# OthmanB/TAMCMC-C

Measured on AMD Instinct MI355X. Metric: MCMC samples/sec (whole node), 1e5 nu-bins x 100 params x 20 tempered chains, higher is better.
Workload: dtype f64

## Files before the change

### tamcmc-c_amd/csrc/dev_sampler.hip

```cpp
#include <hip/hip_runtime.h>

#include <atomic>
#include <chrono>
#include <hip/hip_ext.h>

#include <cmath>
#include <cstdio>
#include <cstdlib>
#include <cstring>
#include <algorithm>
#include <type_traits>
#include <utility>
#include <vector>

#include "ctx.h"
#include "rgb_prestep.h"
#include "dev_sampler.h"
#include "kernels.h"
#include "loglike_tile.h"
#include "dev_unpack.h"
#include "fd_batch.h"
#include "mode_tables.h"
#include "rng.h"
#include "step_schedule.h"

namespace tamcmc {

namespace {

#include "dev_iterate_impl.h"
#include "dev_step_impl.h"
#include "dev_mala_impl.h"

}


struct DevSampler::Impl {
    tamcmc_hip_ctx *ctx = nullptr;
    DevSamplerArgs a{};
    std::vector<void *> allocs;
    hipEvent_t ev[64][2];
    int n_ev = 0;
    bool poly_ready = false;
    double *adapt_scratch = nullptr;
    size_t smp_cap = 0, stat_cap = 0;
    size_t lds_base = 0, lds_adapt = 0;
    int parity = 0;
    FusedArgs f{};
    unsigned char *d_argcopy = nullptr;
    std::vector<unsigned char> h_argcopy;
    bool use_drift = false;
    double delta = 0, fd_step_rel = 1e-7;
    FdBatch fd;
    DevBuf<unsigned char> fd_block;
    DevBuf<double> fd_part, fd_S, fd_model, fd_bg;
    DevBuf<double> fused_bg, fused_part;
    MalaArgs mala{};
    bool grad_valid = false;
    int prior_class = 0, model_id = 0;
    std::vector<double> h_priors, h_extra;
    std::vector<int32_t> h_idx, h_sw;
    long armed_it = -1;
    int armed_q = 0;
    long it_fused = 0, it_lockstep = 0;
    long n_stretch = 0;
    int mala_chol_lds = -1;

    hipEvent_t gev[8][2];
    int n_gev = 0;
    bool rgb = false;
    int rgb_bmax = 0;
    bool fused_ok = false;
    int fused_mode = -1, fused_K = 0;
    int tile_rot = 0;
    std::vector<int32_t> h_plength;
    int G = 1;
    hipStream_t gst[4] = {nullptr, nullptr, nullptr, nullptr};
    hipEvent_t ev_kb[4], ev_ki[4], ev_fork, ev_join[4];
    bool ev_made = false;
    double *d_pack = nullptr, *h_pack = nullptr;

    double *device_view(const double *host, size_t bytes) {
        if (!host || !bytes) return nullptr;
        double *d = nullptr;
        void *dp = nullptr, *dq = nullptr;
        const char *last = (const char *)host + bytes - 1;
        if (hipHostGetDevicePointer(&dp, const_cast<double *>(host), 0) == hipSuccess && dp &&
            hipHostGetDevicePointer(&dq, const_cast<char *>(last), 0) == hipSuccess && dq == (char *)dp + bytes - 1)
            d = (double *)dp;
        else (void)hipGetLastError();
        return d;
    }

    static hipError_t wait_stream(hipStream_t st, bool poll) {
        const auto t0 = std::chrono::steady_clock::now();
        for (int spin = 0; poll; spin++) {
            const hipError_t e = hipStreamQuery(st);
            if (e != hipErrorNotReady) return e;
            if ((spin & 63) == 63 && std::chrono::steady_clock::now() - t0 > std::chrono::microseconds(1000)) break;
        }
        (void)hipGetLastError();
        return hipStreamSynchronize(st);
    }

    template <typename T>
    hipError_t dalloc(T **p, size_t n) {
        void *q = nullptr;
        hipError_t e = hipMalloc(&q, (n ? n : 1) * sizeof(T));
        if (e == hipSuccess) { allocs.push_back(q); *p = (T *)q; }
        return e;
    }

    struct KernelTiming;
    struct RunCall;
};

DevSampler::DevSampler() : impl(new Impl()) {}
DevSampler::~DevSampler() {
    if (!impl) return;
    if (impl->ctx) {
        (void)hipSetDevice(impl->ctx->device);
        (void)hipStreamSynchronize(impl->ctx->stream);
        for (int g = 1; g < 4; g++) if (impl->gst[g]) (void)hipStreamSynchronize(impl->gst[g]);
    }
#ifdef TAMCMC_PROBE
    if (impl->a.counters && getenv("TAMCMC_PROBE_STEP")) {
        long h[40];
        (void)hipMemcpy(h, impl->a.counters + 8 + impl->a.C, sizeof h, hipMemcpyDeviceToHost);
        if (h[35] > 0) fprintf(stderr, "build_multiplet, row 20 (us): decode + widths/heights %.2f | window %.2f | m loop %.2f\n", 0.01 * h[32] / h[35], 0.01 * h[33] / h[35], 0.01 * h[34] / h[35]);
        for (int r = 0; r < 4; r++)
            if (h[8 * r + 3] > 0)
                fprintf(stderr, "candidate role %d of slot 2 (us): decide %.2f | vectors + L z %.2f | role %.2f  [inside: %.2f | %.2f]  (%ld launches)\n", r,
                        0.01 * h[8 * r] / h[8 * r + 3], 0.01 * h[8 * r + 1] / h[8 * r + 3], 0.01 * h[8 * r + 2] / h[8 * r + 3],
                        0.01 * h[8 * r + 4] / h[8 * r + 3], 0.01 * h[8 * r + 5] / h[8 * r + 3], h[8 * r + 3]);
    }
    if (impl->a.counters && getenv("TAMCMC_PROBE_ADAPT")) {
        long h[8];
        (void)hipMemcpy(h, impl->a.counters, sizeof h, hipMemcpyDeviceToHost);
        if (h[7] > 0)
            fprintf(stderr, "Cholesky panels of chain 0 (us per panel): columns below %.2f | next panel's columns %.2f | next diagonal block beside the rest of the trailing update %.2f  (%ld panels)\n",
                    0.01 * h[4] / h[7], 0.01 * h[5] / h[7], 0.01 * h[6] / h[7], h[7]);
    }
#endif
    for (void *p : impl->allocs) (void)hipFree(p);
    impl->fd_block.release(); impl->fd_part.release(); impl->fd_S.release(); impl->fd_model.release(); impl->fd_bg.release(); impl->fused_bg.release(); impl->fused_part.release();
    if (impl->h_pack) (void)hipHostFree(impl->h_pack);
    for (int i = 0; i < impl->n_ev; i++) { (void)hipEventDestroy(impl->ev[i][0]); (void)hipEventDestroy(impl->ev[i][1]); }
    for (int i = 0; i < impl->n_gev; i++) { (void)hipEventDestroy(impl->gev[i][0]); (void)hipEventDestroy(impl->gev[i][1]); }
    if (impl->ev_made) {
        (void)hipEventDestroy(impl->ev_fork);
        for (int g = 0; g < 4; g++) { (void)hipEventDestroy(impl->ev_kb[g]); (void)hipEventDestroy(impl->ev_ki[g]); (void)hipEventDestroy(impl->ev_join[g]); }
        for (int g = 1; g < 4; g++) if (impl->gst[g]) (void)hipStreamDestroy(impl->gst[g]);
    }
    delete impl;
}

#define DCHK(call)                                                                   \
    do {                                                                             \
        hipError_t e_ = (call);                                                      \
        if (e_ != hipSuccess) {                                                      \
            c->err = std::string(#call) + ": " + hipGetErrorString(e_);              \
            return TAMCMC_ERR_HIP;                                                   \
        }                                                                            \
    } while (0)

template <typename T>
static hipError_t up(T *dst, const T *src, size_t n, hipStream_t st) {
    return hipMemcpyAsync(dst, src, n * sizeof(T), hipMemcpyHostToDevice, st);
}

int DevSampler::init(tamcmc_hip_ctx *c, const DevSamplerInit &in) {
    Impl &I = *impl;
    I.ctx = c;
    if (c->Nx <= 0) return TAMCMC_ERR_NO_SPECTRUM;
    if (in.C < 1 || in.C > TAMCMC_MAX_CHAINS) return TAMCMC_ERR_BAD_ARG;
    DCHK(hipSetDevice(c->device));
    DevSamplerArgs &a = I.a;
    a.desc.model_id = in.model_id; a.desc.prior_class = in.prior_class; a.C = in.C; a.desc.Np = in.Np; a.Nv = in.Nv;
    I.rgb = is_rgb_model(in.model_id);
#ifdef TAMCMC_PROBE
    if (const char *ep = getenv("TAMCMC_PROBE_ADAPT")) a.probe = atoi(ep);
#endif
    a.desc.per = I.rgb ? 0 : mt::count_multiplets(in.model_id, in.plength);
    I.h_plength.assign(in.plength, in.plength + 11);
    I.use_drift = in.use_drift != 0; I.delta = in.delta; I.fd_step_rel = in.fd_step_rel > 0 ? in.fd_step_rel : 1e-7;
    I.prior_class = in.prior_class; I.model_id = in.model_id;
    I.h_priors.assign(in.priors, in.priors + 4 * (size_t)in.Np); I.h_extra.assign(in.extra_priors, in.extra_priors + 10);
    I.h_idx.assign(in.index_to_relax, in.index_to_relax + in.Nv); I.h_sw.assign(in.priors_switch, in.priors_switch + in.Np);
    if (a.desc.per < 0) return TAMCMC_ERR_BAD_MODEL;
    a.desc.stride = in.plength[8] > 0 ? in.plength[8] : 1;
    if ((a.desc.stride - 1) / 3 > TAMCMC_MAX_HARVEY) return TAMCMC_ERR_BAD_ARG;
    {
        int G = in.chain_groups > 0 ? in.chain_groups : (in.C >= 8 ? 2 : 1);
        if (in.chain_groups <= 0 && I.rgb && in.C >= 16) G = 4;
        if (G > 4) G = 4;
        if (G > in.C) G = in.C;
        I.G = G;
    }
// ... 34 lines not shown
    DCHK(I.dalloc(&a.noise, CD * (size_t)a.desc.stride));
    DCHK(hipMemsetAsync(a.counters, 0, (8 + C + 64) * sizeof(long), st));
    DCHK(hipMemsetAsync(a.moved, 0, C * sizeof(int), st));
    DCHK(hipMemsetAsync(a.Pmove, 0, C * sizeof(double), st));
    a.samples = nullptr; a.stats = nullptr;
    I.lds_base = (Np + 2 * Nv + 1) * sizeof(double) + unpack_lds_bytes() + 32;
    I.lds_adapt = (Nv * Nv + Nv) * sizeof(double);
    a.chol_in_lds = (I.lds_base + I.lds_adapt <= 150 * 1024) ? 1 : 0;
    if (!a.chol_in_lds) { DCHK(I.dalloc(&I.adapt_scratch, C * (Nv * Nv + Nv))); I.lds_adapt = 0; }
    if (I.lds_base + I.lds_adapt > 64 * 1024) {
        DCHK(hipFuncSetAttribute((const void *)k_iterate<true>, hipFuncAttributeMaxDynamicSharedMemorySize, (int)(I.lds_base + I.lds_adapt)));
        DCHK(hipFuncSetAttribute((const void *)k_iterate<false>, hipFuncAttributeMaxDynamicSharedMemorySize, (int)(I.lds_base + I.lds_adapt)));
    }
    mt::PolyTab *d_tab;
    DCHK(I.dalloc(&d_tab, 1));
    hipLaunchKernelGGL(k_fill_poly, dim3(1), dim3(64), 0, st, d_tab);
    DCHK(hipGetLastError());
    a.desc.poly = d_tab;
    for (int i = 0; i < 64; i++) { DCHK(hipEventCreate(&I.ev[i][0])); DCHK(hipEventCreate(&I.ev[i][1])); I.n_ev = i + 1; }
    for (int i = 0; i < 8; i++) { DCHK(hipEventCreate(&I.gev[i][0])); DCHK(hipEventCreate(&I.gev[i][1])); I.n_gev = i + 1; }
    {
        const int G = I.G;
        I.gst[0] = st;
        for (int g = 1; g < G; g++) DCHK(hipStreamCreateWithFlags(&I.gst[g], hipStreamNonBlocking));
        DCHK(hipEventCreateWithFlags(&I.ev_fork, hipEventDisableTiming));
        for (int g = 0; g < 4; g++) {
            DCHK(hipEventCreateWithFlags(&I.ev_kb[g], hipEventDisableTiming));
            DCHK(hipEventCreateWithFlags(&I.ev_ki[g], hipEventDisableTiming));
            DCHK(hipEventCreateWithFlags(&I.ev_join[g], hipEventDisableTiming));
        }
        I.ev_made = true;
    }
    {
        FusedArgs &f = I.f;
        f.NS = 2 * in.C + 8;
        {
            const int h = (int)(((long)in.C * 1) / 2);
            f.xsplit = (I.G == 2 && h >= 3 && in.C - h >= 3) ? h : in.C;
        }
        const size_t NS = (size_t)f.NS;
        DCHK(I.dalloc(&f.cand_vars, 3 * NS * Nv)); DCHK(I.dalloc(&f.cand_params, 3 * NS * Np)); DCHK(I.dalloc(&f.cand_logPr, 6 * NS));
        DCHK(I.dalloc(&f.cand_stP, 6 * NS)); DCHK(I.dalloc(&f.cand_stR, 3 * NS)); DCHK(I.dalloc(&f.cand_rej, 3 * NS));
        DCHK(I.dalloc(&f.mults, 3 * NS * (size_t)a.desc.per + 1)); DCHK(I.dalloc(&f.pairs, 6 * NS)); DCHK(I.dalloc(&f.nh, 3 * NS)); DCHK(I.dalloc(&f.nn, 3 * NS));
        DCHK(I.dalloc(&f.noise, 3 * NS * (size_t)a.desc.stride));
        DCHK(I.dalloc(&f.slot, 2 * C)); DCHK(I.dalloc(&f.prop_logPr, 2 * C)); DCHK(I.dalloc(&f.prop_st, 2 * C)); DCHK(I.dalloc(&f.quick, 2 * C * QN)); DCHK(I.dalloc(&f.lz, 2 * C * Nv));
        DCHK(I.dalloc(&f.qcount, 2));
        DCHK(hipMemsetAsync(f.qcount, 0, 2 * sizeof(unsigned long long), st));
        f.qmargin = 1e-11;
        DCHK(hipMemsetAsync(f.nn, 0, 3 * NS * sizeof(int), st));
        DCHK(hipMemsetAsync(f.cand_stP, 0, 6 * NS * sizeof(int), st));
        DCHK(hipMemsetAsync(f.cand_rej, 0, 3 * NS * sizeof(int), st));
        DCHK(hipMemsetAsync(f.cand_stR, 0, 3 * NS * sizeof(int), st));
        f.part = nullptr;
        f.bg = nullptr;
        const size_t role_lds = (Np + 2 * Nv + 1) * sizeof(double) + unpack_lds_bytes() + 32;
        I.fused_ok = !I.rgb && role_lds <= sizeof(tile::TileLds<tile::M_FAST_DIRECT, 64>);
    }
    DCHK(hipStreamSynchronize(st));
    return TAMCMC_OK;
}

int DevSampler::download_gradient(double *grad, double *grad_prior) {
    Impl &I = *impl;
    tamcmc_hip_ctx *c = I.ctx;
    if (!I.use_drift || !I.a.grad_cur || !I.grad_valid) return TAMCMC_ERR_BAD_ARG;
    DCHK(hipSetDevice(c->device));
    const size_t n = (size_t)I.a.C * I.a.Nv;
    DCHK(hipStreamSynchronize(c->stream));
    if (grad) DCHK(hipMemcpy(grad, I.a.grad_cur + (size_t)I.parity * n, n * sizeof(double), hipMemcpyDeviceToHost));
    if (grad_prior) DCHK(hipMemcpy(grad_prior, I.a.gradP_cur + (size_t)I.parity * n, n * sizeof(double), hipMemcpyDeviceToHost));
    return TAMCMC_OK;
}

int DevSampler::download_last_proposal(double *vars_prop, double *grad_prop) {
    Impl &I = *impl;
    tamcmc_hip_ctx *c = I.ctx;
    if (!I.use_drift) return TAMCMC_ERR_BAD_ARG;
    DCHK(hipSetDevice(c->device));
    const size_t n = (size_t)I.a.C * I.a.Nv;
    DCHK(hipStreamSynchronize(c->stream));
    if (vars_prop) DCHK(hipMemcpy(vars_prop, I.a.vars_prop, n * sizeof(double), hipMemcpyDeviceToHost));
    if (grad_prop) DCHK(hipMemcpy(grad_prop, I.mala.grad_prop, n * sizeof(double), hipMemcpyDeviceToHost));
    return TAMCMC_OK;
}

void DevSampler::info(long out[11]) const {
    const Impl &I = *impl;
    unsigned long long qc[2] = {0, 0};
    if (I.f.qcount && hipSetDevice(I.ctx->device) == hipSuccess) (void)hipMemcpy(qc, I.f.qcount, sizeof qc, hipMemcpyDeviceToHost);
    out[8] = I.n_stretch; out[9] = (long)qc[0]; out[10] = (long)qc[1];
    out[0] = I.a.Nv; out[1] = I.a.desc.Np;
    out[2] = I.use_drift ? I.mala_chol_lds : I.a.chol_in_lds;
    out[3] = (I.fused_ok && !I.use_drift) ? 1 : 0;
    out[4] = I.G; out[5] = I.it_fused; out[6] = I.it_lockstep; out[7] = I.a.C;
}

int DevSampler::upload_state(const double *vars, const double *params, const double *logL, const double *logPr,
                             const double *logPost, const double *init_logL) {
    Impl &I = *impl;
    I.armed_it = -1;
    I.grad_valid = false;
    tamcmc_hip_ctx *c = I.ctx;
    DevSamplerArgs &a = I.a;
    const size_t C = (size_t)a.C, Np = (size_t)a.desc.Np, Nv = (size_t)a.Nv;
    hipStream_t st = c->stream;
    DCHK(hipSetDevice(c->device));
// ... 204 lines not shown
    return e;
}

struct DevSampler::Impl::RunCall {
    Impl &I;
    tamcmc_hip_ctx *c;
    DevSamplerArgs &a;
    const long it0, n_iter;
    const char *learn;
    double *samples, *stats;
    hipStream_t st;
    CallTimeline &tl;
    KernelTiming T;
    DevSamplerArgs args;
    LoglikeArgs la[4], lf[3];
    int goff[5];
    double *zc_smp = nullptr, *zc_st = nullptr;
    bool use_fused = false;
    bool split_ok = false;
    int P;
    StepCtl sc{};
    int q = 0;
    bool s1_must_wait = false;
    bool s1_ahead = false;
    bool s1_open = false;

    RunCall(Impl &I_, CallTimeline &tl_, long it0_, long n_iter_, const char *learn_, double *samples_, double *stats_)
        : I(I_), c(I_.ctx), a(I_.a), it0(it0_), n_iter(n_iter_), learn(learn_), samples(samples_), stats(stats_), st(I_.ctx->stream),
          tl(tl_), T{I_, I_.ctx}, P(I_.parity) {}

    int prepare() {
        const size_t C = (size_t)a.C, Nv = (size_t)a.Nv;
        const int tb = tile_bins(c->wgs, c->K);
        a.ntiles = (a.desc.Nx + tb - 1) / tb;
        DCHK(c->d_part.reserve(C * (size_t)a.ntiles * 2));
        a.partials = c->d_part.p;
        a.tile_bins = tb;
        a.bg = nullptr;
        use_fused = I.fused_ok && c->step_scheme != 1 && c->wgs == 64 && (c->K == 4 || c->K == 8 || c->K == 16);
        I.f.qmargin = c->quick_decide == 1 ? (double)INFINITY : 1e-11;
        const size_t NS = (size_t)I.f.NS;
        I.f.bg = nullptr;
        if (c->precision == TAMCMC_PRECISION_FAST) {
            DCHK(c->d_bg.reserve(C * (size_t)a.ntiles * 8));
            a.bg = c->d_bg.p;
            if (use_fused) {
                DCHK(I.fused_bg.reserve(3 * NS * (size_t)a.ntiles * 8));
                I.f.bg = I.fused_bg.p;
            }
        }
        if (use_fused) {
            DCHK(I.fused_part.reserve(2 * C * (size_t)a.ntiles * 2));
            I.f.part = I.fused_part.p;
        }
        split_ok = I.f.xsplit < a.C && c->step_scheme != 2 && (c->step_scheme == 3 || (long)a.C * a.ntiles >= 2500);
        auto grown = [](size_t need, size_t have, size_t unit) { const size_t floor_ = 256 * unit; return std::max(std::max(need, floor_), have * 2); };
        zc_smp = I.device_view(samples, (size_t)n_iter * C * Nv * 8);
        zc_st = I.device_view(stats, (size_t)n_iter * C * 3 * 8);
        if (samples && !zc_smp && I.smp_cap < (size_t)n_iter * C * Nv) {
            const size_t cap = grown((size_t)n_iter * C * Nv, I.smp_cap, C * Nv);
            DCHK(I.dalloc(&a.samples, cap));
            I.smp_cap = cap;
        }
        if (stats && !zc_st && I.stat_cap < (size_t)n_iter * C * 3) {
            const size_t cap = grown((size_t)n_iter * C * 3, I.stat_cap, C * 3);
            DCHK(I.dalloc(&a.stats, cap));
            I.stat_cap = cap;
        }
        args = a;
        args.samples = samples ? (zc_smp ? zc_smp : a.samples) : nullptr;
        args.stats = stats ? (zc_st ? zc_st : a.stats) : nullptr;
        const int G = I.G;
        for (int g = 0; g <= G; g++) goff[g] = (int)(((long)a.C * g) / G);
        auto fill_common = [&](LoglikeArgs &l, int B) {
            l.x = c->dx.p; l.y = c->dy.p; l.logx = c->dlogx.p; l.Nx = a.desc.Nx; l.B = B; l.ntiles = a.ntiles;
            l.x0 = a.desc.x_first; l.step = a.desc.step; l.noise_stride = a.desc.stride; l.model = nullptr; l.tile_rot = I.tile_rot;
        };
        for (int g = 0; g < G; g++) {
            LoglikeArgs &l = la[g];
            const int first = goff[g];
            fill_common(l, goff[g + 1] - goff[g]);
            l.mults = a.mults; l.offsets = a.pairs + 2 * first; l.noise = a.noise + (size_t)first * a.desc.stride;
            l.per = a.desc.per; l.slot0 = first;
            l.nharvey = a.nh + first; l.nnoise = a.nn + first; l.partials = a.partials + (size_t)first * a.ntiles * 2;
            l.bg_poly = a.bg ? a.bg + (size_t)first * a.ntiles * 8 : nullptr;
        }
        for (int e = 0; e < 3; e++) {
            LoglikeArgs &l = lf[e];
            const FusedArgs &f = I.f;
            fill_common(l, a.C);
            l.mults = f.mults + (size_t)e * NS * a.desc.per; l.offsets = f.pairs + (size_t)e * 2 * NS; l.noise = f.noise + (size_t)e * NS * a.desc.stride;
            l.nharvey = f.nh + (size_t)e * NS; l.nnoise = f.nn + (size_t)e * NS; l.partials = f.part;
            l.bg_poly = f.bg ? f.bg + (size_t)e * NS * a.ntiles * 8 : nullptr;
            l.per = a.desc.per; l.slot0 = 0;
        }
        return TAMCMC_OK;
    }

    int swap_pair_of(long it) const { return swap_pair(a.seed, a.C, a.dN_mixing, it, nullptr); }

    int run_lockstep(long ia, long ib) {
        const int G = I.G;
        const size_t C = (size_t)a.C;
        I.armed_it = -1;
        I.it_lockstep += ib - ia;
        if (G > 1) {
// ... 356 lines not shown
```

### tamcmc-c_amd/csrc/dev_step_impl.h

```cpp

struct FusedArgs {
    int NS;
    int xsplit;
    double *cand_vars, *cand_params;
    double *cand_logPr;
    int *cand_rej;
    int *cand_stP, *cand_stR;
    tamcmc_multiplet *mults;
    int *pairs, *nh, *nn;
    double *noise;
    double *bg;
    int *slot;
    double *prop_logPr;
    int *prop_st;
    double *quick;
    double *part;
    double *lz;
    double qmargin;
    unsigned long long *qcount;
};

constexpr int QN = 8;
constexpr int ST_L = 1, ST_BR = 2, ST_ENTRY = 4, ST_LZ = 8, ST_FIRST = 16, ST_COMMIT = 32;

typedef DevSamplerArgs __attribute__((address_space(4))) ConstArgs;
typedef FusedArgs __attribute__((address_space(4))) ConstFused;
__device__ __forceinline__ const void __attribute__((address_space(4))) *uniform_ptr(const void *p) {
    const unsigned long long v = (unsigned long long)p;
    const unsigned lo = (unsigned)__builtin_amdgcn_readfirstlane((int)(v & 0xffffffffull)), hi = (unsigned)__builtin_amdgcn_readfirstlane((int)(v >> 32));
    return (const void __attribute__((address_space(4))) *)(((unsigned long long)hi << 32) | lo);
}

struct Decided {
    int slot;
    int src;
    int src_acc;
    int src_par;
    int src_ps;
    int swap_first;
    int swapped;
    double r;
    AcceptOut o;
};

__device__ __attribute__((noinline)) int decide(const DevSamplerArgs *ga, const FusedArgs *gf, int m, long it, int q, int settled, Decided *out) {
    const ConstArgs &a = *(const ConstArgs *)uniform_ptr(ga);
    const ConstFused &f = *(const ConstFused *)uniform_ptr(gf);
    const int lane = threadIdx.x & 63, C = a.C;
    if (settled) {
        const int s = f.slot[q * C + m] & 0xffff;
        if (out && lane == 0) {
            Decided d;
            d.slot = s; d.src = m; d.src_acc = 0; d.src_par = q; d.src_ps = 0; d.swap_first = -1; d.swapped = 0; d.r = 0;
            d.o.acc = 0; d.o.r = 0; d.o.logL = 0; d.o.logPr = 0; d.o.logPost = 0;
            *out = d;
        }
        return s;
    }
    const int p = q ^ 1, ntiles = a.ntiles;
    const long itp = it - 1;
    int A = -1;
    double u = 0;
    if (is_swap_iter(a, itp)) A = swap_first(a, itp, &u);
    const bool in_pair = A >= 0 && (m == A || m == A + 1);
    const int j0 = in_pair ? A : m;
    const int jl = (in_pair && lane == 1) ? A + 1 : j0;
    const int ps = f.slot[p * C + jl] & 0xffff, st = f.prop_st[p * C + jl];
    const double pl = f.prop_logPr[p * C + jl], hL = a.logL_cur[p * C + jl], hP = a.logPr_cur[p * C + jl], hQ = a.logPost_cur[p * C + jl];
    const double Tj = a.Tcoefs[jl], il = a.init_logL[jl];
// ... 70 lines not shown
        rng_uniform2(a.seed, RNG_ACCEPT, (uint32_t)m, (uint64_t)it, 0, u, u1);
        if (stm == TAMCMC_OK && !(lp == -INFINITY || isnan(lp))) {
            const double cur = settled ? a.logPost_cur[q * C + m] : d.o.logPost;
            Sstar = -((log(u) - lp + cur) * Tm) / (double)a.pl;
            if (isfinite(Sstar)) ok = 1;
        } else if (u > 0.0) ok = 2;
        w[0] = Sstar; w[1] = ok; w[2] = -(double)a.pl / Tm; w[3] = settled ? a.logL_cur[q * C + m] : d.o.logL;
        double lus = 0, k1 = 0, k2 = 0;
        if (is_swap_iter(a, it)) {
            double us;
            if (swap_first(a, it, &us) == m) {
                const double TB = a.Tcoefs[m + 1];
                lus = log(us); k1 = Tm / TB - 1.0; k2 = TB / Tm - 1.0;
            }
        }
        w[4] = lus; w[5] = k1; w[6] = k2; w[7] = (double)slot;
    }
    if (settled) return;
    const double *sv, *sp;
    if (d.src_acc) {
        const size_t gp = (size_t)((it - 1) % 3) * f.NS + d.src_ps;
        sv = f.cand_vars + gp * Nv;
        sp = f.cand_params + gp * Np;
    } else {
        sv = a.vars_cur + ((size_t)d.src_par * C + d.src) * Nv;
        sp = a.params_cur + ((size_t)d.src_par * C + d.src) * Np;
    }
    double *dv = a.vars_cur + ((size_t)q * C + m) * Nv, *dp = a.params_cur + ((size_t)q * C + m) * Np;
    double *rv = (a.samples && rec >= 0) ? a.samples + ((size_t)rec * C + m) * Nv : nullptr;
    for (int i = lane; i < Nv; i += 64) { const double v = sv[i]; dv[i] = v; if (rv) rv[i] = v; }
    for (int i = lane; i < Np; i += 64) dp[i] = sp[i];
    if (lane == 0) {
        a.logL_cur[q * C + m] = d.o.logL;
        a.logPr_cur[q * C + m] = d.o.logPr;
        a.logPost_cur[q * C + m] = d.o.logPost;
        f.slot[q * C + m] = slot;
        a.moved[m] = d.src_acc;
        a.Pmove[m] = d.r;
        if (m == 0 && d.src_acc) a.counters[1] += 1;
        a.counters[8 + m] += d.src_acc;
        if (m == 0) a.counters[0] = it;
        if (d.swap_first == m) {
            atomicAdd((unsigned long long *)&a.counters[2], 1ull);
            if (d.swapped) atomicAdd((unsigned long long *)&a.counters[3], 1ull);
        }
        if (a.stats && rec >= 0) {
            double *r = a.stats + ((size_t)rec * C + m) * 3;
            r[0] = d.o.logL; r[1] = d.o.logPr; r[2] = d.o.logPost;
        }
        if (tiles && d.swap_first < 0 && f.quick[((size_t)(q ^ 1) * C + m) * QN + 1] == 2.0) atomicAdd(f.qcount + 1, 1ull);
    }
}

__device__ __attribute__((noinline)) int quick_decide_leaf(const DevSamplerArgs *ga, const FusedArgs *gf, int m, int q, int pairA, Decided *out) {
    const ConstArgs &a = *(const ConstArgs *)uniform_ptr(ga);
    const ConstFused &f = *(const ConstFused *)uniform_ptr(gf);
    const int lane = threadIdx.x & 63, C = a.C;
    const int p = q ^ 1, n2 = 2 * a.ntiles;
    const bool in_pair = pairA >= 0 && (m == pairA || m == pairA + 1);
    const int j0 = in_pair ? pairA : m;
    const double *b0 = f.part + ((size_t)p * C + j0) * n2;
    const double *r0 = f.quick + ((size_t)p * C + j0) * QN;
    const double rec = (lane < (in_pair ? 2 * QN : QN)) ? r0[lane] : 0.0;
    double s0 = 0, a0 = 0, s1 = 0, a1 = 0;
    for (int t0 = 0; t0 < n2; t0 += 512) {
        double v[8], w[8];
#pragma unroll
        for (int k = 0; k < 8; k++) {
            const int t = t0 + k * 64 + lane;
            v[k] = t < n2 ? b0[t] : 0.0;
            w[k] = (in_pair && t < n2) ? b0[n2 + t] : 0.0;
        }
#pragma unroll
        for (int k = 0; k < 8; k++) { s0 += v[k]; a0 += fabs(v[k]); s1 += w[k]; a1 += fabs(w[k]); }
    }
#pragma unroll
    for (int off = 32; off >= 1; off >>= 1) { s0 += __shfl_xor(s0, off, 64); a0 += __shfl_xor(a0, off, 64); }
    if (in_pair) {
#pragma unroll
        for (int off = 32; off >= 1; off >>= 1) { s1 += __shfl_xor(s1, off, 64); a1 += __shfl_xor(a1, off, 64); }
    }
    const double St0 = __shfl(rec, 0, 64), ok0 = __shfl(rec, 1, 64);
    const int ps0 = (int)__shfl(rec, 7, 64);
    const double mg = f.qmargin;
    int acc0 = 0;
    if (ok0 == 2.0) { s0 = 0; a0 = 0; }
    else if (ok0 > 0 && fabs(s0 - St0) > mg * (a0 + fabs(St0))) acc0 = s0 < St0 ? 1 : 0;
    else return -1;
    Decided d;
    d.swap_first = -1; d.swapped = 0; d.src_par = p; d.r = 0;
    d.o.acc = 0; d.o.r = 0; d.o.logL = 0; d.o.logPr = 0; d.o.logPost = 0;
    if (!in_pair) { d.slot = 2 * m + acc0; d.src = m; d.src_acc = acc0; d.src_ps = ps0; }
    else {
        const double St1 = __shfl(rec, QN, 64), ok1 = __shfl(rec, QN + 1, 64);
        const int ps1 = (int)__shfl(rec, QN + 7, 64);
        int acc1 = 0;
        if (ok1 == 2.0) { s1 = 0; a1 = 0; }
        else if (ok1 > 0 && fabs(s1 - St1) > mg * (a1 + fabs(St1))) acc1 = s1 < St1 ? 1 : 0;
        else return -1;
        const double c0 = __shfl(rec, 2, 64), c1 = __shfl(rec, QN + 2, 64);
        const double LA = acc0 ? c0 * s0 : __shfl(rec, 3, 64), LB = acc1 ? c1 * s1 : __shfl(rec, QN + 3, 64);
        const double lus = __shfl(rec, 4, 64), x = LA * __shfl(rec, 5, 64) + LB * __shfl(rec, 6, 64);
        if (!(fabs(x - lus) > mg * (fabs(c0) * a0 + fabs(c1) * a1 + fabs(LA) + fabs(LB)))) return -1;
        const int swapped = x > lus ? 1 : 0;
        const int A = pairA, B = pairA + 1;
        d.swap_first = A; d.swapped = swapped;
        if (swapped) {
            if (m == A) { d.slot = 2 * C + (A >= f.xsplit ? 4 : 0) + acc1; d.src = B; d.src_acc = acc1; d.src_ps = ps1; }
            else { d.slot = 2 * C + (B >= f.xsplit ? 4 : 0) + 2 + acc0; d.src = A; d.src_acc = acc0; d.src_ps = ps0; }
        } else {
            if (m == A) { d.slot = 2 * A + acc0; d.src = A; d.src_acc = acc0; d.src_ps = ps0; }
            else { d.slot = 2 * B + acc1; d.src = B; d.src_acc = acc1; d.src_ps = ps1; }
        }
    }
    if (out && lane == 0) *out = d;
    return d.slot;
}

__device__ __forceinline__ int quick_decide(const DevSamplerArgs *ga, const FusedArgs *gf, int m, long it, int q, int settled, int pairA,
                                            Decided *out) {
    if (settled) return decide(ga, gf, m, it, q, 1, out);
    const int s = quick_decide_leaf(ga, gf, m, q, pairA, out);
    return s >= 0 ? s : decide(ga, gf, m, it, q, 0, out);
}

__device__ __attribute__((noinline)) int decide_counted(const DevSamplerArgs *ga, const FusedArgs *gf, int m, long it, int q, int tile) {
    if (tile == 0 && (threadIdx.x & 63) == 0) atomicAdd(((const ConstFused *)uniform_ptr(gf))->qcount, 1ull);
    return decide(ga, gf, m, it, q, 0, nullptr);
}
__device__ __forceinline__ int quick_slot(const DevSamplerArgs *ga, const FusedArgs *gf, int m, long it, int q, int settled, int pairA, int tile) {
    if (settled) return decide(ga, gf, m, it, q, 1, nullptr);
    const int s = quick_decide_leaf(ga, gf, m, q, pairA, nullptr);
    return s >= 0 ? s : decide_counted(ga, gf, m, it, q, tile);
}

struct StepTiles {
    const DevSamplerArgs *ga;
    const FusedArgs *gf;
    long it;
    int q, first, settled, pairA;
    static constexpr bool coherent_partials = false;
    __device__ __forceinline__ int slot(const LoglikeArgs &, int b, int tile) const { return quick_slot(ga, gf, first + b, it, q, settled, pairA, tile); }
    __device__ __forceinline__ void operator()(int, int, int) const {}
};

__device__ __attribute__((noinline)) void role_prior(const DevSamplerArgs *ga, const FusedArgs *gf, size_t gs, int h, const double *s_vars,
                                                     const double *s_params, const UnpackLds *Up) {
    const DevSamplerArgs &a = *ga;
    const FusedArgs &f = *gf;
    const UnpackLds U = *Up;
    const int Nv = a.Nv, Np = a.desc.Np, tid = threadIdx.x;
    if (h == 0) {
        for (int i = tid; i < Nv; i += 64) f.cand_vars[gs * Nv + i] = s_vars[i];
        for (int i = tid; i < Np; i += 64) f.cand_params[gs * Np + i] = s_params[i];
    }
    int rej = 0;
#ifdef TAMCMC_PROBE
    long ps_[4] = {0, 0, 0, 0};
    const double fh = wave_log_prior_part(a.desc, s_params, U, TB - 128, h, &rej, ps_);
    if (tid == 0 && (int)(gs % f.NS) == 2) { long *w = a.counters + 8 + a.C + 16 * h + 4; w[0] += ps_[1] - ps_[0]; w[1] += ps_[2] - ps_[1]; }
#else
    const double fh = wave_log_prior_part(a.desc, s_params, U, TB - 128, h, &rej);
#endif
    if (tid == 0) {
        f.cand_logPr[2 * gs + h] = fh;
        f.cand_stP[2 * gs + h] = *U.status;
        if (h == 0) f.cand_rej[gs] = rej;
    }
}
__device__ __forceinline__ TablePtrs candidate_tables(const DevSamplerArgs &a, const FusedArgs &f, int q_dst) {
    TablePtrs T;
    T.mults = f.mults + (size_t)q_dst * f.NS * a.desc.per; T.pairs = f.pairs + (size_t)q_dst * 2 * f.NS; T.nh = f.nh + (size_t)q_dst * f.NS;
    T.nn = f.nn + (size_t)q_dst * f.NS; T.noise = f.noise + (size_t)q_dst * f.NS * a.desc.stride;
    T.bg = nullptr; T.ntiles = a.ntiles; T.tile_bins = a.tile_bins;
    return T;
}
__device__ __attribute__((noinline)) void role_rows(const DevSamplerArgs *ga, const FusedArgs *gf, int q_dst, int slot, size_t gs,
                                                    const double *s_params, const UnpackLds *Up) {
    const DevSamplerArgs &a = *ga;
    const FusedArgs &f = *gf;
    const UnpackLds U = *Up;
    if (threadIdx.x == 0) mt::shared_scalars_base(a.desc.model_id, s_params, a.desc.plength, *U.S);
    __syncthreads();
    const TablePtrs T = candidate_tables(a, f, q_dst);
#ifdef TAMCMC_PROBE
    __shared__ long ps_[8];
    wg_unpack(a.desc, s_params, U, slot, T, true, false, false, true, ps_);
    __syncthreads();
    if (threadIdx.x == 0 && (int)(gs % f.NS) == 2) {
        long *w = a.counters + 8 + a.C + 8 + 4; w[0] += ps_[1] - ps_[0]; w[1] += ps_[2] - ps_[1];
        long *v = a.counters + 8 + a.C + 32; v[0] += ps_[5] - ps_[4]; v[1] += ps_[6] - ps_[5]; v[2] += ps_[7] - ps_[6]; v[3] += 1;
    }
#else
    wg_unpack(a.desc, s_params, U, slot, T, true, false, false, true);
#endif
// ... 200 lines not shown
```

### tamcmc-c_amd/csrc/loglike_tile.h

```cpp
#pragma once
#include <hip/hip_runtime.h>
#include <stdint.h>

#include "kernels.h"
#include "bg_series.h"

namespace tamcmc {
namespace tile {

constexpr int CHUNK = 64;

constexpr int F_FULL = 1;
constexpr int F_SAFE = 2;
constexpr int F_ASYM = 4;
constexpr int F_FAR = 8;

constexpr int M_STRICT = 0, M_FAST_DIRECT = 2, M_FAST = 1;

constexpr int NC = 16;
constexpr double RHO_MAX2 = 1.0 / 36.0;
constexpr double RHO_MAX2_ASYM = 1.0 / 64.0;
constexpr int NH = bg::NH;
constexpr int ROW = NC + 2;

// ... 126 lines not shown
                acc[k] = acc[k] + res;
            }
            if (K > 4 && (k & 3) == 3) __builtin_amdgcn_sched_barrier(0);
        }
    } else {
#pragma unroll
        for (int k = 0; k < K; k++) {
            if (FULL || (bin[k] >= i0 && bin[k] < i1)) {
                const double xx = xv[k];
                const double dx = xx - xc;
                double res = 0.0;
#pragma unroll
                for (int m = 0; m < NM; m++) {
                    const double t = fma(dx, g, nA[m]);
                    res = res + hv[m] / fma(t, t, 1.0);
                }
                if (flags & F_ASYM) {
                    const double ta = fma(M.fcx, xx, 1.0 - M.asym);
                    res = res * fma(ta, ta, M.c2sq);
                }
                acc[k] = acc[k] + res;
            }
        }
    }
}

template <bool FAST, int NM, int K>
__device__ __forceinline__ void mult_dispatch(const LdsMult &M, const double (&xv)[K], const int (&bin)[K], double (&acc)[K], double xc) {
    if (M.flags & F_FULL) {
        if (FAST) fast_mult<NM, K, true>(M, xv, bin, acc, xc);
        else strict_mult<NM, K, true>(M, xv, bin, acc);
    } else {
        if (FAST) fast_mult<NM, K, false>(M, xv, bin, acc, xc);
        else strict_mult<NM, K, false>(M, xv, bin, acc);
    }
}


template <int MODE, int WGS>
struct __attribute__((aligned(16))) TileLds {
    static constexpr bool FARFIELD = (MODE == M_FAST);
    static constexpr int LDS_BYTES = FARFIELD ? (WGS * ROW * 8 > CHUNK * (int)sizeof(LdsMult) ? WGS * ROW * 8 : CHUNK * (int)sizeof(LdsMult))
                                              : CHUNK * (int)sizeof(LdsMult);
    unsigned char buf[LDS_BYTES];
    double coef[NC];
    double part[WGS / 16][NC];
    double red[2 * (WGS / 64)];
    double lt[TAMCMC_MAX_HARVEY];
    double lto[TAMCMC_MAX_HARVEY];
    int n, nfar, anyfar;
    unsigned short slot[CHUNK * 7];
};

template <int MODE, int WGS, int K, bool WRITE_MODEL, bool DELTA, bool COH = false>
__device__ __forceinline__ void tile_compute(const LoglikeArgs &a, const int tile, const int b, const int sb, TileLds<MODE, WGS> &S, const int mbeg,
                                             const int mend, const int nh, const int nn) {
    constexpr bool FAST = (MODE != M_STRICT);
    static_assert(!DELTA || (FAST && !WRITE_MODEL), "DELTA launches are FAST-mode, logL-only");
    constexpr bool FARFIELD = (MODE == M_FAST);
    LdsMult *s_m = (LdsMult *)S.buf;
    double *s_rows = (double *)S.buf;
    int &s_n = S.n, &s_nfar = S.nfar, &s_anyfar = S.anyfar;
    unsigned short *s_slot = S.slot;
    double *s_coef = S.coef;
    double(*s_part)[NC] = S.part;
    double *s_red = S.red;
    double *s_lt = S.lt, *s_lto = S.lto;
    const int tid = threadIdx.x;
#ifdef TAMCMC_PROBE
#define KSTAMP(k) do { if (a.dbg && b == 0 && tile == a.ntiles / 2 && tid == 0) a.dbg[k] = (long)wall_clock64(); } while (0)
#define PROBE_SKIP(bit) (a.probe & (bit))
    const long wg_t0 = (a.dbg && a.dbg[7] == 77) ? (long)wall_clock64() : 0;
#else
#define KSTAMP(k) do { } while (0)
#define PROBE_SKIP(bit) false
#endif
    KSTAMP(0);
    constexpr int TILE = WGS * K;
    const int t0 = tile * TILE;
    const int t1 = min(t0 + TILE, a.Nx);
    if (DELTA) {
        if (a.d_done && a.d_done[(size_t)b * a.ntiles + tile]) return;
        const int lo = a.d_range[2 * b], hi = a.d_range[2 * b + 1];
        if (t1 <= lo || t0 >= hi) {
            if (tid == 0) {
                double *p = a.partials + ((size_t)b * a.ntiles + tile) * 2;
                p[0] = 0.0;
                p[1] = 0.0;
            }
            return;
        }
    }

    tamcmc_multiplet g;
    const bool fullnew = DELTA && (a.d_flags[b] & 2);
    const bool dsub = DELTA && !fullnew;
    const bool bg_prebuilt = FARFIELD && a.bg_poly && (!DELTA || fullnew);
    double bg_pre = 0.0;
    if (bg_prebuilt && tid < NH) bg_pre = a.bg_poly[((size_t)(DELTA ? a.d_row[b] : sb) * a.ntiles + tile) * NH + tid];
    double xv[K], yv[K], acc[K];
    int bin[K];
#pragma unroll
    for (int k = 0; k < K; k++) {
        bin[k] = t0 + k * WGS + tid;
        const int bi = min(bin[k], a.Nx - 1);
        xv[k] = a.x[bi];
        acc[k] = 0.0;
    }

    const double *nz = a.noise + (size_t)sb * a.noise_stride;
    const bool bg = !DELTA || fullnew || (a.d_flags[b] & 1);
    const double *nzo = DELTA ? a.d_noise_old + (size_t)b * a.noise_stride : nz;
    const double h = 0.5 * (double)TILE * a.step;
    const double xc = a.x0 + ((double)t0 + 0.5 * (double)TILE - 0.5) * a.step;
    const bool harvey_poly = FARFIELD && bg && bg::series_valid(xc, h);
    if (FAST && bg && !harvey_poly) {
        if (tid < nh) {
            s_lt[tid] = log(1e-3 * nz[3 * tid + 1]);
            if (dsub) s_lto[tid] = log(1e-3 * nzo[3 * tid + 1]);
        }
    }
    if (FARFIELD) {
        if (tid < NC) s_coef[tid] = 0.0;
        if (tid == 0) s_anyfar = harvey_poly ? 1 : 0;
        __syncthreads();
        if (harvey_poly && !bg_prebuilt) {
            const int hl = (WGS > 64) ? tid - 64 : tid;
            double f[NH];
#pragma unroll
            for (int k = 0; k < NH; k++) f[k] = 0.0;
            const bool lane_new = (hl >= 0 && hl < nh), lane_old = dsub && (hl >= 32 && hl < 32 + nh);
            if (lane_new || lane_old) {
                const double *nq = lane_new ? nz : nzo;
                const int ht = lane_new ? hl : hl - 32;
                bg::harvey_term_series(lane_new ? nq[3 * ht] : -nq[3 * ht], nq[3 * ht + 1], nq[3 * ht + 2], xc, h, f);
            }
            if (hl >= 0 && hl < 64) {
#pragma unroll
                for (int k = 0; k < NH; k++) {
                    double v = f[k];
                    double tot = 0.0;
                    for (int t = 0; t < nh; t++) tot = tot + __shfl(v, t, 64);
                    if (dsub)
                        for (int t = 0; t < nh; t++) tot = tot + __shfl(v, 32 + t, 64);
                    const double wn = dsub ? (nz[nn - 1] - nzo[nn - 1]) : nz[nn - 1];
                    if (hl == 0) s_coef[k] = tot + (k == 0 ? wn : 0.0);
                }
            }
        }
    }

    bool bg_in_regs = harvey_poly && bg_prebuilt;
    bool any_near = false;
    KSTAMP(1);
    for (int c0 = mbeg; c0 < mend; c0 += CHUNK) {
        __syncthreads();
        if (tid < 64) {
            const int idx = c0 + tid;
            g = a.mults[a.per > 0 ? min(idx, mbeg + a.per - 1) : min(idx, mend - 1)];
// ... 246 lines not shown
                    double pz = fma(u, 0.2 - yr, yr - 0.25);
                    pz = fma(u, pz, (1.0 / 3.0) - yr);
                    pz = fma(u, pz, yr - 0.5);
                    pz = fma(u, pz, 1.0 - yr);
                    f = u * pz;
                } else f = fma(-yr * u, rcp_nr2(1.0 + u), log1p(u));
                if (valid) s[0] = s[0] + f;
            } else if (valid) {
                if (PROBE_SKIP(8)) s[0] = s[0] + yv[k] * Mv;
                else {
                    ynum = fma(ynum, Mv, yv[k] * prod);
                    prod = prod * Mv;
                }
            }
        }
        Mk[k] = Mv;
        if (WRITE_MODEL) {
            if (valid) {
                if (a.fd_rows) {
                    const double r0 = FAST ? rcp_nr2(Mv) : 1.0 / Mv;
                    a.fd_rows[(size_t)b * a.Nx + bin[k]] = r0;
                    a.fd_rows[a.fd_plane + (size_t)b * a.Nx + bin[k]] = yv[k] * r0;
                    a.fd_rows[2 * a.fd_plane + (size_t)b * a.Nx + bin[k]] = Mv;
                } else a.model[(size_t)b * a.Nx + bin[k]] = Mv;
            }
        }
    }
    if (FAST && !DELTA) {
        if (prod > 1e-280 && prod < 1e280) {
            s[1] = log(prod);
            s[0] = s[0] + ynum * rcp_nr2(prod);
        } else {
#pragma unroll
            for (int k = 0; k < K; k++)
                if (bin[k] < a.Nx) {
                    s[1] = s[1] + log(Mk[k]);
                    s[0] = fma(yv[k], rcp_nr2(Mk[k]), s[0]);
                }
        }
    }
    __syncthreads();
    double out[2];
    block_reduce<2, WGS>(s, s_red, out);
    if (tid == 0) {
        double *p = a.partials + ((size_t)b * a.ntiles + tile) * 2;
        if (COH) {
            typedef double __attribute__((address_space(1))) *gdp_t;
            __hip_atomic_store((gdp_t)p, out[0], __ATOMIC_RELAXED, __HIP_MEMORY_SCOPE_AGENT);
            __hip_atomic_store((gdp_t)p + 1, out[1], __ATOMIC_RELAXED, __HIP_MEMORY_SCOPE_AGENT);
        } else {
            p[0] = out[0];
            p[1] = out[1];
        }
    }
    KSTAMP(6);
#ifdef TAMCMC_PROBE
    if (a.dbg && a.dbg[7] == 77 && tid == 0) {
        long *w = a.dbg + 8 + 2 * ((size_t)b * a.ntiles + tile);
        w[0] = wg_t0;
        w[1] = (long)wall_clock64();
    }
#endif
#undef KSTAMP
#undef PROBE_SKIP
}

struct NoTail {
    static constexpr bool coherent_partials = false;
    __device__ __forceinline__ int slot(const LoglikeArgs &, int b, int ) const { return b; }
    __device__ __forceinline__ void operator()(int , int , int ) const {}
};

template <int MODE, int WGS, int K, bool WRITE_MODEL, bool DELTA, class Tail>
__device__ __forceinline__ void loglike_tile(const LoglikeArgs &a, const int id, TileLds<MODE, WGS> &S, const Tail &tail) {
    const int xcd = id & 7;
    int j = id >> 3, b, tile;
    if (a.prio_b < 0) {
        b = j % a.B;
        tile = (j / a.B) * 8 + xcd;
    } else {
        const int lead = ((a.ntiles + 7) >> 3) * 2;
        if (j < lead) {
            b = a.prio_b + (j & 1);
            tile = (j >> 1) * 8 + xcd;
        } else {
            j -= lead;
            const int rest = a.B - 2, r = j % rest;
            b = r + (r >= a.prio_b ? 2 : 0);
            tile = (j / rest) * 8 + xcd;
        }
    }
    if (tile >= a.ntiles) return;
    tile += a.tile_rot;
    if (tile >= a.ntiles) tile -= a.ntiles;
    const int sb = tail.slot(a, b, tile);
    const int nn = a.nnoise[sb], nh = a.nharvey[sb];
    const int mend = a.offsets[2 * sb + 1];
    const int mbeg = a.per > 0 ? (a.slot0 + sb) * a.per : a.offsets[2 * sb];
    if (nn > 0)
        tile_compute<MODE, WGS, K, WRITE_MODEL, DELTA, Tail::coherent_partials>(a, tile, b, sb, S, mbeg, mend, nh, nn);
    tail(b, tile, sb);
}

}
}
```

Measured before the change: 47650.

## Store per-tile summed partials and prefetch slot words and x before quick decide

Each tile now also writes the sum of its two partials into a new psum buffer. The quick decision then reads half as many values (ntiles instead of 2*ntiles) per chain, and reads the pair only when needed, via a templated reduction. For step tiles, the x values and the slot metadata for both candidate slots are loaded before the quick decide, so their latency overlaps the decision. The cost is one extra global store per tile, a new buffer, and some extra speculative loads.

```diff
diff --git a/tamcmc-c_amd/csrc/dev_sampler.hip b/tamcmc-c_amd/csrc/dev_sampler.hip
--- a/tamcmc-c_amd/csrc/dev_sampler.hip
+++ b/tamcmc-c_amd/csrc/dev_sampler.hip
@@ -54,7 +54,7 @@
     FdBatch fd;
     DevBuf<unsigned char> fd_block;
     DevBuf<double> fd_part, fd_S, fd_model, fd_bg;
-    DevBuf<double> fused_bg, fused_part;
+    DevBuf<double> fused_bg, fused_part, fused_psum;
     MalaArgs mala{};
     bool grad_valid = false;
     int prior_class = 0, model_id = 0;
@@ -143,7 +143,7 @@
     }
 #endif
     for (void *p : impl->allocs) (void)hipFree(p);
-    impl->fd_block.release(); impl->fd_part.release(); impl->fd_S.release(); impl->fd_model.release(); impl->fd_bg.release(); impl->fused_bg.release(); impl->fused_part.release();
+    impl->fd_block.release(); impl->fd_part.release(); impl->fd_S.release(); impl->fd_model.release(); impl->fd_bg.release(); impl->fused_bg.release(); impl->fused_part.release(); impl->fused_psum.release();
     if (impl->h_pack) (void)hipHostFree(impl->h_pack);
     for (int i = 0; i < impl->n_ev; i++) { (void)hipEventDestroy(impl->ev[i][0]); (void)hipEventDestroy(impl->ev[i][1]); }
     for (int i = 0; i < impl->n_gev; i++) { (void)hipEventDestroy(impl->gev[i][0]); (void)hipEventDestroy(impl->gev[i][1]); }
@@ -284,6 +284,7 @@
         DCHK(hipMemsetAsync(f.cand_rej, 0, 3 * NS * sizeof(int), st));
         DCHK(hipMemsetAsync(f.cand_stR, 0, 3 * NS * sizeof(int), st));
         f.part = nullptr;
+        f.psum = nullptr;
         f.bg = nullptr;
         const size_t role_lds = (Np + 2 * Nv + 1) * sizeof(double) + unpack_lds_bytes() + 32;
         I.fused_ok = !I.rgb && role_lds <= sizeof(tile::TileLds<tile::M_FAST_DIRECT, 64>);
@@ -594,6 +595,8 @@
         if (use_fused) {
             DCHK(I.fused_part.reserve(2 * C * (size_t)a.ntiles * 2));
             I.f.part = I.fused_part.p;
+            DCHK(I.fused_psum.reserve(2 * C * (size_t)a.ntiles));
+            I.f.psum = I.fused_psum.p;
         }
         split_ok = I.f.xsplit < a.C && c->step_scheme != 2 && (c->step_scheme == 3 || (long)a.C * a.ntiles >= 2500);
         auto grown = [](size_t need, size_t have, size_t unit) { const size_t floor_ = 256 * unit; return std::max(std::max(need, floor_), have * 2); };
diff --git a/tamcmc-c_amd/csrc/dev_step_impl.h b/tamcmc-c_amd/csrc/dev_step_impl.h
--- a/tamcmc-c_amd/csrc/dev_step_impl.h
+++ b/tamcmc-c_amd/csrc/dev_step_impl.h
@@ -15,6 +15,7 @@
     int *prop_st;
     double *quick;
     double *part;
+    double *psum;
     double *lz;
     double qmargin;
     unsigned long long *qcount;
@@ -191,33 +192,45 @@
     }
 }
 
-__device__ __attribute__((noinline)) int quick_decide_leaf(const DevSamplerArgs *ga, const FusedArgs *gf, int m, int q, int pairA, Decided *out) {
+
+template <bool PAIR>
+__device__ __forceinline__ void quick_sums(const double *c0, int n, int lane, double &s0, double &a0, double &s1, double &a1) {
+    for (int t0 = 0; t0 < n; t0 += 256) {
+        double v[4], w[4];
+#pragma unroll
+        for (int k = 0; k < 4; k++) {
+            const int t = t0 + k * 64 + lane;
+            v[k] = t < n ? c0[t] : 0.0;
+            if (PAIR) w[k] = t < n ? c0[n + t] : 0.0;
+        }
+#pragma unroll
+        for (int k = 0; k < 4; k++) {
+            s0 += v[k]; a0 += fabs(v[k]);
+            if (PAIR) { s1 += w[k]; a1 += fabs(w[k]); }
+        }
+    }
+#pragma unroll
+    for (int off = 32; off >= 1; off >>= 1) {
+        s0 += __shfl_xor(s0, off, 64); a0 += __shfl_xor(a0, off, 64);
+        if (PAIR) { s1 += __shfl_xor(s1, off, 64); a1 += __shfl_xor(a1, off, 64); }
+    }
+}
+__device__ __forceinline__ int quick_decide_core(const DevSamplerArgs *ga, const FusedArgs *gf, int m, int q, int pairA, Decided *out) {
     const ConstArgs &a = *(const ConstArgs *)uniform_ptr(ga);
     const ConstFused &f = *(const ConstFused *)uniform_ptr(gf);
     const int lane = threadIdx.x & 63, C = a.C;
-    const int p = q ^ 1, n2 = 2 * a.ntiles;
+    const int p = q ^ 1, n = a.ntiles;
     const bool in_pair = pairA >= 0 && (m == pairA || m == pairA + 1);
     const int j0 = in_pair ? pairA : m;
-    const double *b0 = f.part + ((size_t)p * C + j0) * n2;
+    const double *c0 = f.psum + ((size_t)p * C + j0) * n;
     const double *r0 = f.quick + ((size_t)p * C + j0) * QN;
-    const double rec = (lane < (in_pair ? 2 * QN : QN)) ? r0[lane] : 0.0;
-    double s0 = 0, a0 = 0, s1 = 0, a1 = 0;
-    for (int t0 = 0; t0 < n2; t0 += 512) {
-        double v[8], w[8];
-#pragma unroll
-        for (int k = 0; k < 8; k++) {
-            const int t = t0 + k * 64 + lane;
-            v[k] = t < n2 ? b0[t] : 0.0;
-            w[k] = (in_pair && t < n2) ? b0[n2 + t] : 0.0;
-        }
-#pragma unroll
-        for (int k = 0; k < 8; k++) { s0 += v[k]; a0 += fabs(v[k]); s1 += w[k]; a1 += fabs(w[k]); }
-    }
-#pragma unroll
-    for (int off = 32; off >= 1; off >>= 1) { s0 += __shfl_xor(s0, off, 64); a0 += __shfl_xor(a0, off, 64); }
+    double rec, s0 = 0, a0 = 0, s1 = 0, a1 = 0;
     if (in_pair) {
-#pragma unroll
-        for (int off = 32; off >= 1; off >>= 1) { s1 += __shfl_xor(s1, off, 64); a1 += __shfl_xor(a1, off, 64); }
+        rec = lane < 2 * QN ? r0[lane] : 0.0;
+        quick_sums<true>(c0, n, lane, s0, a0, s1, a1);
+    } else {
+        rec = lane < QN ? r0[lane] : 0.0;
+        quick_sums<false>(c0, n, lane, s0, a0, s1, a1);
     }
     const double St0 = __shfl(rec, 0, 64), ok0 = __shfl(rec, 1, 64);
     const int ps0 = (int)__shfl(rec, 7, 64);
@@ -255,6 +268,9 @@
     if (out && lane == 0) *out = d;
     return d.slot;
 }
+__device__ __attribute__((noinline)) int quick_decide_leaf(const DevSamplerArgs *ga, const FusedArgs *gf, int m, int q, int pairA, Decided *out) {
+    return quick_decide_core(ga, gf, m, q, pairA, out);
+}
 
 __device__ __forceinline__ int quick_decide(const DevSamplerArgs *ga, const FusedArgs *gf, int m, long it, int q, int settled, int pairA,
                                             Decided *out) {
@@ -266,11 +282,6 @@
 __device__ __attribute__((noinline)) int decide_counted(const DevSamplerArgs *ga, const FusedArgs *gf, int m, long it, int q, int tile) {
     if (tile == 0 && (threadIdx.x & 63) == 0) atomicAdd(((const ConstFused *)uniform_ptr(gf))->qcount, 1ull);
     return decide(ga, gf, m, it, q, 0, nullptr);
-}
-__device__ __forceinline__ int quick_slot(const DevSamplerArgs *ga, const FusedArgs *gf, int m, long it, int q, int settled, int pairA, int tile) {
-    if (settled) return decide(ga, gf, m, it, q, 1, nullptr);
-    const int s = quick_decide_leaf(ga, gf, m, q, pairA, nullptr);
-    return s >= 0 ? s : decide_counted(ga, gf, m, it, q, tile);
 }
 
 struct StepTiles {
@@ -279,7 +290,23 @@
     long it;
     int q, first, settled, pairA;
     static constexpr bool coherent_partials = false;
-    __device__ __forceinline__ int slot(const LoglikeArgs &, int b, int tile) const { return quick_slot(ga, gf, first + b, it, q, settled, pairA, tile); }
+    static constexpr bool early_loads = true;
+    __device__ __forceinline__ tile::SlotWords head(const LoglikeArgs &a, int b, int tile) const {
+        const int m = first + b;
+        if (settled) return tile::slot_words(a, decide(ga, gf, m, it, q, 1, nullptr));
+        const bool lone = a.per > 0 && !(pairA >= 0 && (m == pairA || m == pairA + 1));
+        tile::SlotWords w0{}, w1{};
+        if (lone) { w0 = tile::slot_words(a, 2 * m); w1 = tile::slot_words(a, 2 * m + 1); }
+        int s = quick_decide_core(ga, gf, m, q, pairA, nullptr);
+        if (s < 0) s = decide_counted(ga, gf, m, it, q, tile);
+        if (lone && (s >> 1) == m) return (s & 1) ? w1 : w0;
+        return tile::slot_words(a, s);
+    }
+    __device__ __forceinline__ void store_sums(int b, int tile, double s0, double s1) const {
+        const ConstArgs &a = *(const ConstArgs *)uniform_ptr(ga);
+        const ConstFused &f = *(const ConstFused *)uniform_ptr(gf);
+        f.psum[((size_t)q * a.C + first + b) * a.ntiles + tile] = s0 + s1;
+    }
     __device__ __forceinline__ void operator()(int, int, int) const {}
 };
 
diff --git a/tamcmc-c_amd/csrc/loglike_tile.h b/tamcmc-c_amd/csrc/loglike_tile.h
--- a/tamcmc-c_amd/csrc/loglike_tile.h
+++ b/tamcmc-c_amd/csrc/loglike_tile.h
@@ -202,10 +202,11 @@
     unsigned short slot[CHUNK * 7];
 };
 
-template <int MODE, int WGS, int K, bool WRITE_MODEL, bool DELTA, bool COH = false>
+template <int MODE, int WGS, int K, bool WRITE_MODEL, bool DELTA, class Tail>
 __device__ __forceinline__ void tile_compute(const LoglikeArgs &a, const int tile, const int b, const int sb, TileLds<MODE, WGS> &S, const int mbeg,
-                                             const int mend, const int nh, const int nn) {
+                                             const int mend, const int nh, const int nn, const Tail &tail, const double *xpre) {
     constexpr bool FAST = (MODE != M_STRICT);
+    constexpr bool COH = Tail::coherent_partials;
     static_assert(!DELTA || (FAST && !WRITE_MODEL), "DELTA launches are FAST-mode, logL-only");
     constexpr bool FARFIELD = (MODE == M_FAST);
     LdsMult *s_m = (LdsMult *)S.buf;
@@ -254,7 +255,7 @@
     for (int k = 0; k < K; k++) {
         bin[k] = t0 + k * WGS + tid;
         const int bi = min(bin[k], a.Nx - 1);
-        xv[k] = a.x[bi];
+        xv[k] = xpre ? xpre[k] : a.x[bi];
         acc[k] = 0.0;
     }
 
@@ -607,6 +608,7 @@
             p[0] = out[0];
             p[1] = out[1];
         }
+        tail.store_sums(b, tile, out[0], out[1]);
     }
     KSTAMP(6);
 #ifdef TAMCMC_PROBE
@@ -620,9 +622,20 @@
 #undef PROBE_SKIP
 }
 
+struct SlotWords { int sb, nn, nh, mbeg, mend; };
+__device__ __forceinline__ SlotWords slot_words(const LoglikeArgs &a, int sb) {
+    SlotWords w;
+    w.sb = sb; w.nn = a.nnoise[sb]; w.nh = a.nharvey[sb];
+    w.mend = a.offsets[2 * sb + 1];
+    w.mbeg = a.per > 0 ? (a.slot0 + sb) * a.per : a.offsets[2 * sb];
+    return w;
+}
+
 struct NoTail {
     static constexpr bool coherent_partials = false;
+    static constexpr bool early_loads = false;
     __device__ __forceinline__ int slot(const LoglikeArgs &, int b, int ) const { return b; }
+    __device__ __forceinline__ void store_sums(int , int , double, double) const {}
     __device__ __forceinline__ void operator()(int , int , int ) const {}
 };
 
@@ -648,14 +661,17 @@
     if (tile >= a.ntiles) return;
     tile += a.tile_rot;
     if (tile >= a.ntiles) tile -= a.ntiles;
-    const int sb = tail.slot(a, b, tile);
-    const int nn = a.nnoise[sb], nh = a.nharvey[sb];
-    const int mend = a.offsets[2 * sb + 1];
-    const int mbeg = a.per > 0 ? (a.slot0 + sb) * a.per : a.offsets[2 * sb];
-    if (nn > 0)
-        tile_compute<MODE, WGS, K, WRITE_MODEL, DELTA, Tail::coherent_partials>(a, tile, b, sb, S, mbeg, mend, nh, nn);
-    tail(b, tile, sb);
-}
-
-}
-}
+    SlotWords w;
+    double xpre[Tail::early_loads ? K : 1];
+    if constexpr (Tail::early_loads) {
+#pragma unroll
+        for (int k = 0; k < K; k++) xpre[k] = a.x[min(tile * (WGS * K) + k * WGS + (int)threadIdx.x, a.Nx - 1)];
+        w = tail.head(a, b, tile);
+    } else w = slot_words(a, tail.slot(a, b, tile));
+    if (w.nn > 0)
+        tile_compute<MODE, WGS, K, WRITE_MODEL, DELTA, Tail>(a, tile, b, w.sb, S, w.mbeg, w.mend, w.nh, w.nn, tail, Tail::early_loads ? xpre : nullptr);
+    tail(b, tile, w.sb);
+}
+
+}
+}
```

Result: faster. 48880, median of 6 (+2.6%).
